# vivek87799/lightweight-human-pose-estimation.pytorch

Hardware: AMD Instinct MI355X
Metric: frames/sec end-to-end (net+grouping) at 368px (higher is better)
Workload: dtype f32; 1 GPU; batch=1 per GPU, 368x656 frames, 1 refinement stage(s), fp32 convs / f32+f64 post, resident normalised NCHW input -> key-points + pose entries on host; 3 frame batch(es) in flight per GPU (3 engine stream(s), each step a complete pass); global_batch=1, parallelism=dp1 (frames sharded, no data-path collective), 3 stream(s) per GPU

## Files before the change

lightweight-human-pose-estimation.pytorch_amd/csrc/net_kernels.hip:

```cpp
#include <cstdio>
#include <cstdlib>

#include <type_traits>
#include "lwp_internal.h"

namespace lwp {

typedef float f32x4 __attribute__((ext_vector_type(4)));
typedef float f32x2 __attribute__((ext_vector_type(2)));
typedef float f32x16 __attribute__((ext_vector_type(16)));

__device__ __forceinline__ float elu_negative(float v) {
    const float p = v * (1.f + v * (0.5f + v * (1.f / 6.f + v * (1.f / 24.f + v * (1.f / 120.f + v * (1.f / 720.f + v * (1.f / 5040.f)))))));
    return v > -0.5f ? p : __expf(v) - 1.0f;
}
__device__ __forceinline__ float apply_act(float v, int act) {
    if (act == ACT_RELU) return fmaxf(v, 0.0f);
    if (act == ACT_ELU) return v > 0.0f ? v : elu_negative(v);
    return v;
}

constexpr int ST_TX = 32;
template <bool BF16, int ST_TY, int PY = 1, int DBG = 0, bool WL = false, bool F16 = false>
__global__ void __launch_bounds__(ST_TY * ST_TX) stem_kernel(StemParams p) {
// ... 1070 lines not shown
                    *(f32x4*)(At + (row0 + i) * ldA + c) = acc;
                }
            } else {
                int xi = xo, yi = yo, im = img;
#pragma unroll
                for (int i = 0; i < PXG; ++i) {
                    const bool ok = m + i < M32;
                    const int yc = yi * p.stride, xc = xi * p.stride;
                    const int base = ((im * p.Hi + yc) * p.Wi + xc) * pix_b + c * 4;
                    f32x4 x[9];
#pragma unroll
                    for (int t = 0; t < 9; ++t) {
                        const int dy = (t / 3 - 1) * p.dil, dx = (t % 3 - 1) * p.dil;
                        const bool in = ok && yc + dy >= 0 && yc + dy < p.Hi && xc + dx >= 0 && xc + dx < p.Wi;
                        x[t] = ldw(in ? (unsigned)(base + dy * row_b + dx * pix_b) : 0x80000000u);
                    }
                    f32x4 acc = bias;
#pragma unroll
                    for (int t = 0; t < 9; ++t) acc += x[t] * wv[t];
                    acc.x = apply_act(acc.x, act_dw); acc.y = apply_act(acc.y, act_dw);
                    acc.z = apply_act(acc.z, act_dw); acc.w = apply_act(acc.w, act_dw);
                    *(f32x4*)(At + (row0 + i) * ldA + c) = acc;
                    if (++xi == Wo) { xi = 0; if (++yi == Ho) { yi = 0; ++im; } }
                }
            }
            m += adv;
            xo += adv_x; yo += adv_y;
            if (xo >= Wo) { xo -= Wo; ++yo; }
            while (yo >= Ho) { yo -= Ho; ++img; }
        }
    }
    __syncthreads();

    f32x4 acc[RT][2];
#pragma unroll
    for (int a = 0; a < RT; ++a) { acc[a][0] = f32x4{0.f, 0.f, 0.f, 0.f}; acc[a][1] = f32x4{0.f, 0.f, 0.f, 0.f}; }
    const float* a_lane = At + r16 * ldA + 4 * q;
    auto one = [&](int step, auto P_) {
        constexpr int P = decltype(P_)::value;
        const int nxt = step + PF - 1 < nsteps ? step + PF - 1 : nsteps - 1;
        if (!(DBG & 2)) load_b(nxt, bw[(P + PF - 1) % PF]);
        __builtin_amdgcn_sched_barrier(0);
        if (DBG & 4) return;
        const f32x4* bcur = bw[P];
#pragma unroll
        for (int u = 0; u < 2; ++u) {
            f32x4 av[RT];
#pragma unroll
            for (int a = 0; a < RT; ++a) av[a] = *(const f32x4*)(a_lane + a * 16 * ldA + step * 32 + 16 * u);
#pragma unroll
            for (int j = 0; j < 4; ++j) {
#pragma unroll
                for (int t = 0; t < 2; ++t) {
                    const int v = u * 8 + j * 2 + t;
                    const float b = bcur[v >> 2][v & 3];
#pragma unroll
                    for (int a = 0; a < RT; ++a) acc[a][t] = __builtin_amdgcn_mfma_f32_16x16x4f32(b, av[a][j], acc[a][t], 0, 0, 0);
                }
            }
        }
    };
    int s0 = 0;
    for (; s0 + PF <= nsteps; s0 += PF) {
        one(s0, std::integral_constant<int, 0>{});
        if (PF > 1) one(s0 + 1, std::integral_constant<int, 1 % PF>{});
        if (PF > 2) one(s0 + 2, std::integral_constant<int, 2 % PF>{});
    }
    if (s0 < nsteps) { one(s0, std::integral_constant<int, 0>{}); ++s0; }
    if (PF > 2 && s0 < nsteps) { one(s0, std::integral_constant<int, 1 % PF>{}); ++s0; }
#pragma unroll
    for (int t = 0; t < 2; ++t) {
        const int n = wave * 32 + t * 16 + 4 * q;
        const f32x4 bias = *(const f32x4*)(p.pw_b + n);
#pragma unroll
        for (int a = 0; a < RT; ++a) {
            const int64_t m = m0 + a * 16 + r16;
            if (m < M) {
                f32x4 v = acc[a][t] + bias;
                v.x = apply_act(v.x, act_pw); v.y = apply_act(v.y, act_pw);
                v.z = apply_act(v.z, act_pw); v.w = apply_act(v.w, act_pw);
                if (p.res) v += *(const f32x4*)(p.res + m * p.res_ld + n);
                *(f32x4*)(p.out + m * p.out_ld + n) = v;
            }
        }
    }
}

template <int BM, int NW, int DBG = 0, int ACT = -1>
static hipError_t launch_dwpw_t(const DwPwParams& p, hipStream_t s) {
    const int64_t M = (int64_t)p.N * p.Ho * p.Wo;
    const size_t lds = (size_t)BM * (p.C + DWPW_F32_APAD) * sizeof(float);
    if ((int64_t)p.N * p.Hi * p.Wi * p.in_ld * 4 >= (1ll << 31)) return hipErrorInvalidValue;
    const int nsplit = (p.cout / 32) / NW;
    static LdsAttrOnce attr;
    if (lds > 48 * 1024) {
        hipError_t e = attr.ensure((const void*)dwpw_kernel<BM, NW, DBG, ACT>, 160 * 1024);
        if (e != hipSuccess) return e;
    }
    hipLaunchKernelGGL((dwpw_kernel<BM, NW, DBG, ACT>), dim3((unsigned)((M + BM - 1) / BM), nsplit), dim3(NW * 64), lds, s, p);
    return hipGetLastError();
}

template <int C>
__global__ void __launch_bounds__(1024) dwpw_pipe_kernel(DwPwParams p, int ntiles) {
    constexpr int BM = 32, NT = 1024, RT = BM / 16, NSTEP = C / 32;
    constexpr int ldA = C + DWPW_F32_APAD;
    constexpr int CG = C / 4;
    constexpr int PAR = NT / CG;
    constexpr int NIT = BM / PAR;
    static_assert(NIT * 4 == NSTEP, "one pixel per four K steps");
    extern __shared__ __attribute__((aligned(16))) float dsm[];
    float* Wd = dsm + 2 * BM * ldA;
    const int tid = threadIdx.x, lane = tid & 63;
    const int wave_u = __builtin_amdgcn_readfirstlane(tid >> 6);
    const int r16 = lane & 15, q = lane >> 4;
    const int M32 = p.N * p.Ho * p.Wo;
    const int G = gridDim.x;
    int bid = blockIdx.x;
    {
        const int qq = G >> 3, rem = G & 7, xcd = bid & 7;
        bid = (xcd < rem ? xcd * (qq + 1) : rem * (qq + 1) + (xcd - rem) * qq) + (bid >> 3);
    }
    for (int i = tid * 4; i < 10 * C; i += NT * 4) *(f32x4*)(Wd + i) = *(const f32x4*)(p.dw_w + i);
    const __amdgpu_buffer_rsrc_t wrsrc = __builtin_amdgcn_make_buffer_rsrc((void*)p.pw_w, 0, 0x7fffffff, 0x00020000);
    const __amdgpu_buffer_rsrc_t irsrc = __builtin_amdgcn_make_buffer_rsrc((void*)p.in, 0, (int)((int64_t)p.N * p.Hi * p.Wi * p.in_ld * 4), 0x00020000);
    const int pix_b = p.in_ld * 4, row_b = p.Wi * pix_b;
    const int c = (tid % CG) * 4, prow = tid / CG;
    constexpr int NU = 16;
    f32x4 bw[2][4];
    auto load_b = [&](int step, f32x4* dst) {
        const unsigned soff = (unsigned)(step * NU + wave_u) * 4096u;
#pragma unroll
        for (int j = 0; j < 4; ++j) dst[j] = __builtin_bit_cast(f32x4, __builtin_amdgcn_raw_buffer_load_b128(wrsrc, lane * 16 + j * 1024, soff, 0));
    };
    f32x4 win[9], pacc;
    auto p_piece = [&](int tl, int it, int j, float* Adst) {
        if (j == 0) {
            const int m = tl * BM + it * PAR + prow;
            const bool ok = m < M32;
            const unsigned q1 = (unsigned)m / (unsigned)p.Wo;
            const int xo = m - (int)q1 * p.Wo;
            const int img = (int)(q1 / (unsigned)p.Ho);
            const int yo = (int)q1 - img * p.Ho;
            const int yc = yo * p.stride, xc = xo * p.stride;
            const int base = ((img * p.Hi + yc) * p.Wi + xc) * pix_b + c * 4;
#pragma unroll
            for (int t = 0; t < 9; ++t) {
                const int dy = (t / 3 - 1) * p.dil, dx = (t % 3 - 1) * p.dil;
                const bool in = ok && yc + dy >= 0 && yc + dy < p.Hi && xc + dx >= 0 && xc + dx < p.Wi;
                win[t] = __builtin_bit_cast(f32x4, __builtin_amdgcn_raw_buffer_load_b128(irsrc, in ? (unsigned)(base + dy * row_b + dx * pix_b) : 0x80000000u, 0, 0));
            }
        } else if (j == 1) {
            pacc = *(const f32x4*)(Wd + 9 * C + c);
#pragma unroll
            for (int t = 0; t < 4; ++t) pacc += win[t] * *(const f32x4*)(Wd + t * C + c);
        } else if (j == 2) {
#pragma unroll
            for (int t = 4; t < 9; ++t) pacc += win[t] * *(const f32x4*)(Wd + t * C + c);
        } else {
            f32x4 v = pacc;
            v.x = fmaxf(v.x, 0.f); v.y = fmaxf(v.y, 0.f); v.z = fmaxf(v.z, 0.f); v.w = fmaxf(v.w, 0.f);
            *(f32x4*)(Adst + (it * PAR + prow) * ldA + c) = v;
        }
    };
    __syncthreads();
    int tile = bid;
    if (tile < ntiles) {
#pragma unroll
        for (int it = 0; it < NIT; ++it)
#pragma unroll
            for (int j = 0; j < 4; ++j) p_piece(tile, it, j, dsm);
    }
    load_b(0, bw[0]);
    __syncthreads();
    int cur = 0;
    for (; tile < ntiles; tile += G) {
        const float* Ac = dsm + cur * BM * ldA;
        float* An = dsm + (cur ^ 1) * BM * ldA;
        const int tnext = tile + G < ntiles ? tile + G : tile;
        f32x4 acc[RT][2];
#pragma unroll
        for (int a = 0; a < RT; ++a) { acc[a][0] = f32x4{0.f, 0.f, 0.f, 0.f}; acc[a][1] = f32x4{0.f, 0.f, 0.f, 0.f}; }
        const float* a_lane = Ac + r16 * ldA + 4 * q;
#pragma unroll
        for (int step = 0; step < NSTEP; ++step) {
            load_b((step + 1) % NSTEP, bw[(step + 1) & 1]);
            __builtin_amdgcn_sched_barrier(0);
            p_piece(tnext, step >> 2, step & 3, An);
            const f32x4* bcur = bw[step & 1];
#pragma unroll
            for (int u = 0; u < 2; ++u) {
                f32x4 av[RT];
#pragma unroll
                for (int a = 0; a < RT; ++a) av[a] = *(const f32x4*)(a_lane + a * 16 * ldA + step * 32 + 16 * u);
#pragma unroll
                for (int j = 0; j < 4; ++j)
#pragma unroll
                    for (int t = 0; t < 2; ++t) {
                        const int v = u * 8 + j * 2 + t;
                        const float b = bcur[v >> 2][v & 3];
#pragma unroll
                        for (int a = 0; a < RT; ++a) acc[a][t] = __builtin_amdgcn_mfma_f32_16x16x4f32(b, av[a][j], acc[a][t], 0, 0, 0);
                    }
            }
        }
        __syncthreads();
        cur ^= 1;
#pragma unroll
        for (int t = 0; t < 2; ++t) {
            const int n = wave_u * 32 + t * 16 + 4 * q;
            const f32x4 bias = *(const f32x4*)(p.pw_b + n);
#pragma unroll
            for (int a = 0; a < RT; ++a) {
                const int m = tile * BM + a * 16 + r16;
                if (m < M32) {
                    f32x4 v = acc[a][t] + bias;
                    v.x = fmaxf(v.x, 0.f); v.y = fmaxf(v.y, 0.f); v.z = fmaxf(v.z, 0.f); v.w = fmaxf(v.w, 0.f);
                    *(f32x4*)(p.out + (int64_t)m * p.out_ld + n) = v;
                }
            }
        }
    }
}

template <int C>
static hipError_t launch_dwpw_pipe_t(const DwPwParams& p, hipStream_t s) {
    const int64_t M = (int64_t)p.N * p.Ho * p.Wo;
    const int ntiles = (int)((M + 31) / 32);
    const size_t lds = (size_t)(2 * 32 * (C + DWPW_F32_APAD) + 10 * C) * sizeof(float);
    static LdsAttrOnce attr;
    hipError_t e = attr.ensure((const void*)dwpw_pipe_kernel<C>, 160 * 1024);
    if (e != hipSuccess) return e;
    int dev = 0, cus = 256;
    if (hipGetDevice(&dev) != hipSuccess || hipDeviceGetAttribute(&cus, hipDeviceAttributeMultiprocessorCount, dev) != hipSuccess || cus <= 0) cus = 256;
    const Tuning& T = p.tune ? *p.tune : default_tuning();
    int grid = cus * (lds <= 80 * 1024 ? 2 : 1);
    if (T.dwpw_pp_grid > 0) grid = T.dwpw_pp_grid;
    if (grid > ntiles) grid = ntiles;
    hipLaunchKernelGGL((dwpw_pipe_kernel<C>), dim3(grid), dim3(1024), lds, s, p, ntiles);
    return hipGetLastError();
}

static hipError_t try_dwpw_pipe(const DwPwParams& p, hipStream_t s, bool* used) {
    *used = false;
    const Tuning& T = p.tune ? *p.tune : default_tuning();
    if (T.dwpw_pipe == 0) return hipSuccess;
    const int64_t M = (int64_t)p.N * p.Ho * p.Wo;
    if (p.cout != 512 || (p.C != 256 && p.C != 512) || p.res || p.act_dw != ACT_RELU || p.act_pw != ACT_RELU) return hipSuccess;
    if ((p.stride != 1 && p.stride != 2) || (p.in_ld & 3) || (p.out_ld & 3) || (((uintptr_t)p.out) & 15) || (((uintptr_t)p.in) & 15)) return hipSuccess;
    if (M >= (1ll << 31) - 64 || (int64_t)p.N * p.Hi * p.Wi * p.in_ld * 4 >= (1ll << 31)) return hipSuccess;
    if (T.dwpw_pipe != 1 && M < 32 * 2048) return hipSuccess;
    if (T.dwpw_pipe != 1 && p.C != 512) return hipSuccess;
    *used = true;
    LWP_VARIANT(p, "dwpw_pipe<%d>", p.C);
    return p.C == 512 ? launch_dwpw_pipe_t<512>(p, s) : launch_dwpw_pipe_t<256>(p, s);
}

bool dwpw_supported(int C, int cout) {
    return C % 32 == 0 && (cout == 64 || cout == 128 || cout == 256 || cout == 512);
}

hipError_t launch_dwpw(const DwPwParams& p_in, hipStream_t s) {
    const DwPwParams& p = p_in;
    {
        bool used = false;
        hipError_t e = try_dwpw_tiled_f32(p, s, &used);
        if (e != hipSuccess || used) return e;
        e = try_dwpw_pipe(p, s, &used);
        if (e != hipSuccess || used) return e;
    }
    const int64_t M = (int64_t)p.N * p.Ho * p.Wo;
    const int nw = p.cout / 32;
    int bm = 16;
    if (M / 32 >= 450) bm = 32;
    if (M / 64 >= 900) bm = 64;
    if (bm == 64 && nw >= 16) bm = 32;
    int nw_wg = nw;
    const Tuning& T = p.tune ? *p.tune : default_tuning();
    if (T.dwpw_bm) bm = T.dwpw_bm;
    if (T.dwpw_nw > 0 && T.dwpw_nw < nw && nw % T.dwpw_nw == 0) nw_wg = T.dwpw_nw;
    if (bm > 64) bm = 64;
    while (bm > 16 && (size_t)bm * (p.C + DWPW_F32_APAD) * sizeof(float) > 150 * 1024) bm >>= 1;
    LWP_VARIANT(p, "dwpw<%d,%d>", bm, nw_wg);
#ifdef LWP_ABLATION
    const int d = T.dwpw_debug;
#define DP_DBG(BM_, NW_, D_) if (bm == BM_ && nw_wg == NW_ && d == D_) return launch_dwpw_t<BM_, NW_, D_>(p, s);
#define DP_DBGS(BM_, NW_) DP_DBG(BM_, NW_, 1) DP_DBG(BM_, NW_, 2) DP_DBG(BM_, NW_, 3) DP_DBG(BM_, NW_, 4) DP_DBG(BM_, NW_, 6) DP_DBG(BM_, NW_, 7) DP_DBG(BM_, NW_, 8)
    DP_DBGS(16, 16) DP_DBGS(16, 8) DP_DBGS(16, 4)
#undef DP_DBGS
#undef DP_DBG
#endif
    const bool relu = p.act_dw == ACT_RELU && p.act_pw == ACT_RELU;
#define DP_CASE(BM_, NW_) if (bm == BM_ && nw_wg == NW_) return relu ? launch_dwpw_t<BM_, NW_, 0, ACT_RELU>(p, s) : launch_dwpw_t<BM_, NW_>(p, s);
    DP_CASE(16, 2) DP_CASE(32, 2) DP_CASE(64, 2)
    DP_CASE(16, 4) DP_CASE(32, 4) DP_CASE(64, 4)
    DP_CASE(16, 8) DP_CASE(32, 8) DP_CASE(64, 8)
    DP_CASE(16, 16) DP_CASE(32, 16) DP_CASE(64, 16)
#undef DP_CASE
    return hipErrorInvalidValue;
}

template <int NW>
__global__ void __launch_bounds__(NW * 64) heads_f32_kernel(HeadsParams p) {
    extern __shared__ __attribute__((aligned(16))) float hsm[];
    const int tid = threadIdx.x, lane = tid & 63;
    const int wave = __builtin_amdgcn_readfirstlane(tid >> 6);
    const int i16 = lane & 15, q = lane >> 4;
    const int M = p.N * p.H * p.W;
    int bid = blockIdx.x;
    {
        const int nwg = gridDim.x, qq = nwg >> 3, rem = nwg & 7, xcd = bid & 7;
        bid = (xcd < rem ? xcd * (qq + 1) : rem * (qq + 1) + (xcd - rem) * qq) + (bid >> 3);
    }
    const int m = bid * 16 + i16;
    const bool mok = m < M;
    const float* in = (const float*)p.in;
    const __amdgpu_buffer_rsrc_t xr = __builtin_amdgcn_make_buffer_rsrc((void*)in, 0, (int)((int64_t)M * p.in_ld * 4), 0x00020000);
    const __amdgpu_buffer_rsrc_t w0r = __builtin_amdgcn_make_buffer_rsrc((void*)p.w0, 0, p.hidden * 128 * 4, 0x00020000);
    const __amdgpu_buffer_rsrc_t w1r = __builtin_amdgcn_make_buffer_rsrc((void*)p.w1, 0, 64 * p.hidden * 4, 0x00020000);
    auto ld = [](const __amdgpu_buffer_rsrc_t& r, unsigned voff, unsigned soff) { return __builtin_bit_cast(f32x4, __builtin_amdgcn_raw_buffer_load_b128(r, voff, soff, 0)); };

    const int ntiles = p.hidden / 16;
    const int my = wave < ntiles ? (ntiles - wave + NW - 1) / NW : 0;
    constexpr int HPF = 3;
    f32x4 w0v[HPF][8], w1v[HPF][4], b0v[HPF];
    const __amdgpu_buffer_rsrc_t b0r = __builtin_amdgcn_make_buffer_rsrc((void*)p.b0, 0, p.hidden * 4, 0x00020000);
    const unsigned w0_lane = (unsigned)(i16 * 128 + 32 * q) * 4u, w1_lane = (unsigned)(i16 * p.hidden + 4 * q) * 4u;
    auto request = [&](int k, f32x4* a, f32x4* b, f32x4* bias) {
        const int ht = wave + (k < my ? k : (my > 0 ? my - 1 : 0)) * NW;
        const int htc = ht < ntiles ? ht : 0;
#pragma unroll
        for (int u = 0; u < 8; ++u) a[u] = ld(w0r, w0_lane + 16u * u, (unsigned)htc * (16u * 128u * 4u));
#pragma unroll
        for (int t = 0; t < 4; ++t) b[t] = ld(w1r, w1_lane + (unsigned)(t * 16 * p.hidden) * 4u, (unsigned)htc * 64u);
        *bias = ld(b0r, 16u * q, (unsigned)htc * 64u);
    };
    request(0, w0v[0], w1v[0], &b0v[0]);
    if (HPF > 2) request(1, w0v[1], w1v[1], &b0v[1]);
    f32x4 xf[8];
#pragma unroll
    for (int u = 0; u < 8; ++u) xf[u] = ld(xr, mok ? (unsigned)((m * p.in_ld + 32 * q + 4 * u) * 4) : 0x80000000u, 0);

    f32x4 acc2[4];
#pragma unroll
    for (int t = 0; t < 4; ++t) acc2[t] = f32x4{0.f, 0.f, 0.f, 0.f};
    const int hsplit = p.out_split > 0 ? p.hidden / 2 : p.hidden;
    const int t_last_lo = p.out_split > 0 ? (p.out_split + 15) / 16 : 4;
    const int t_first_hi = p.out_split > 0 ? p.out_split / 16 : 0;
    auto one = [&](int k, auto P_) {
        constexpr int P = decltype(P_)::value;
        request(k + HPF - 1, w0v[(P + HPF - 1) % HPF], w1v[(P + HPF - 1) % HPF], &b0v[(P + HPF - 1) % HPF]);
        __builtin_amdgcn_sched_barrier(0);
        const f32x4 b0 = b0v[P];
        f32x4 acc1 = {0.f, 0.f, 0.f, 0.f};
#pragma unroll
        for (int u = 0; u < 8; ++u)
#pragma unroll
            for (int c = 0; c < 4; ++c) acc1 = __builtin_amdgcn_mfma_f32_16x16x4f32(w0v[P][u][c], xf[u][c], acc1, 0, 0, 0);
        f32x4 hv;
#pragma unroll
        for (int r = 0; r < 4; ++r) hv[r] = fmaxf(acc1[r] + b0[r], 0.f);
        const int ht = wave + (k < my ? k : 0) * NW;
        const bool first_half = ht * 16 < hsplit;
        const int t_lo = first_half ? 0 : t_first_hi, t_hi = first_half ? t_last_lo : 4;
#pragma unroll
        for (int t = 0; t < 4; ++t) {
            if (t < t_lo || t >= t_hi) continue;
#pragma unroll
            for (int r = 0; r < 4; ++r) acc2[t] = __builtin_amdgcn_mfma_f32_16x16x4f32(w1v[P][t][r], hv[r], acc2[t], 0, 0, 0);
        }
    };
    int k = 0;
    for (; k + HPF <= my; k += HPF) {
        one(k, std::integral_constant<int, 0>{});
        one(k + 1, std::integral_constant<int, 1 % HPF>{});
        if (HPF > 2) one(k + 2, std::integral_constant<int, 2 % HPF>{});
    }
    if (k < my) { one(k, std::integral_constant<int, 0>{}); ++k; }
    if (HPF > 2 && k < my) { one(k, std::integral_constant<int, 1 % HPF>{}); ++k; }

#pragma unroll
    for (int t = 0; t < 4; ++t) *(f32x4*)(hsm + ((wave * 4 + t) * 64 + lane) * 4) = acc2[t];
    __syncthreads();
    if (tid >= 256) return;
    const int t = tid >> 6;
    f32x4 v = *(const f32x4*)(hsm + ((0 * 4 + t) * 64 + lane) * 4);
#pragma unroll
    for (int w = 1; w < NW; ++w) v += *(const f32x4*)(hsm + ((w * 4 + t) * 64 + lane) * 4);
    const int n = 16 * t + 4 * q;
    if (!mok || n >= p.cout) return;
    v += *(const f32x4*)(p.b1 + n);
    float* out = (float*)p.out;
    if (((p.out_ld & 3) == 0) && ((((uintptr_t)out) & 15) == 0) && n + 3 < p.cout) *(f32x4*)(out + (int64_t)m * p.out_ld + n) = v;
    else {
#pragma unroll
        for (int r = 0; r < 4; ++r) if (n + r < p.cout) out[(int64_t)m * p.out_ld + n + r] = v[r];
    }
    if (p.out_nchw || p.out_nchw2) {
        const int HW = p.H * p.W;
        const int img = m / HW, pix = m - img * HW;
        const int c0 = p.out_split > 0 ? p.out_split : p.cout;
#pragma unroll
        for (int r = 0; r < 4; ++r) {
            const int ch = n + r;
            if (ch >= p.cout) continue;
            if (ch < c0) { if (p.out_nchw) p.out_nchw[((int64_t)img * c0 + ch) * HW + pix] = v[r]; }
            else if (p.out_nchw2) p.out_nchw2[((int64_t)img * (p.cout - c0) + (ch - c0)) * HW + pix] = v[r];
        }
    }
}

constexpr int HL_HC = 32, HL_LD0 = 128 + 8, HL_LD1 = HL_HC + 8;
template <int PT>
__global__ void __launch_bounds__(256) heads_f32_lds_kernel(HeadsParams p) {
    extern __shared__ __attribute__((aligned(16))) float hl_sm[];
    float* W0s = hl_sm;
    float* W1s = W0s + 2 * HL_HC * HL_LD0;
    float* B0s = W1s + 2 * 64 * HL_LD1;
    const int tid = threadIdx.x, lane = tid & 63;
    const int wave = __builtin_amdgcn_readfirstlane(tid >> 6);
    const int i16 = lane & 15, q = lane >> 4;
    const int M = p.N * p.H * p.W;
    int bid = blockIdx.x;
    {
        const int nwg = gridDim.x, qq = nwg >> 3, rem = nwg & 7, xcd = bid & 7;
        bid = (xcd < rem ? xcd * (qq + 1) : rem * (qq + 1) + (xcd - rem) * qq) + (bid >> 3);
    }
    int mr[PT];
    bool mok[PT];
#pragma unroll
    for (int i = 0; i < PT; ++i) { mr[i] = bid * (64 * PT) + (wave * PT + i) * 16 + i16; mok[i] = mr[i] < M; }
    const int nch = p.hidden / HL_HC;
    const float* in = (const float*)p.in;
    const __amdgpu_buffer_rsrc_t xr = __builtin_amdgcn_make_buffer_rsrc((void*)in, 0, (int)((int64_t)M * p.in_ld * 4), 0x00020000);
    const __amdgpu_buffer_rsrc_t w0r = __builtin_amdgcn_make_buffer_rsrc((void*)p.w0, 0, p.hidden * 128 * 4, 0x00020000);
    const __amdgpu_buffer_rsrc_t w1r = __builtin_amdgcn_make_buffer_rsrc((void*)p.w1, 0, 64 * p.hidden * 4, 0x00020000);
    auto ld = [](const __amdgpu_buffer_rsrc_t& r, unsigned voff, unsigned soff) { return __builtin_bit_cast(f32x4, __builtin_amdgcn_raw_buffer_load_b128(r, voff, soff, 0)); };
    f32x4 st0[4], st1[2];
    auto request = [&](int c) {
#pragma unroll
        for (int u = 0; u < 4; ++u) {
            const int ch = tid + u * 256, row = ch >> 5, col = (ch & 31) * 4;
            st0[u] = ld(w0r, (unsigned)(row * 128 + col) * 4u, (unsigned)c * (HL_HC * 128 * 4));
        }
#pragma unroll
        for (int u = 0; u < 2; ++u) {
            const int ch = tid + u * 256, row = ch >> 3, col = (ch & 7) * 4;
            st1[u] = ld(w1r, (unsigned)(row * p.hidden + col) * 4u, (unsigned)c * (HL_HC * 4));
        }
    };
    auto land = [&](int buf) {
#pragma unroll
        for (int u = 0; u < 4; ++u) {
            const int ch = tid + u * 256, row = ch >> 5, col = (ch & 31) * 4;
            *(f32x4*)(W0s + (buf * HL_HC + row) * HL_LD0 + col) = st0[u];
        }
#pragma unroll
        for (int u = 0; u < 2; ++u) {
            const int ch = tid + u * 256, row = ch >> 3, col = (ch & 7) * 4;
            *(f32x4*)(W1s + (buf * 64 + row) * HL_LD1 + col) = st1[u];
        }
    };
    request(0);
    f32x4 xf[PT][8];
#pragma unroll
    for (int i = 0; i < PT; ++i)
#pragma unroll
        for (int u = 0; u < 8; ++u) xf[i][u] = ld(xr, mok[i] ? (unsigned)((mr[i] * p.in_ld + 16 * u + 4 * q) * 4) : 0x80000000u, 0);
    for (int i = tid * 4; i < p.hidden; i += 256 * 4) *(f32x4*)(B0s + i) = *(const f32x4*)(p.b0 + i);
    land(0);
    __syncthreads();

    f32x4 acc2[PT][4];
#pragma unroll
    for (int i = 0; i < PT; ++i)
#pragma unroll
        for (int t = 0; t < 4; ++t) acc2[i][t] = f32x4{0.f, 0.f, 0.f, 0.f};
    const int hsplit = p.out_split > 0 ? p.hidden / 2 : p.hidden;
    const int t_last_lo = p.out_split > 0 ? (p.out_split + 15) / 16 : 4;
    const int t_first_hi = p.out_split > 0 ? p.out_split / 16 : 0;
    for (int c = 0; c < nch; ++c) {
        const int buf = c & 1;
        request(c + 1 < nch ? c + 1 : c);
        __builtin_amdgcn_sched_barrier(0);
#pragma unroll
        for (int j = 0; j < HL_HC / 16; ++j) {
            const float* w0 = W0s + (buf * HL_HC + j * 16 + i16) * HL_LD0 + 4 * q;
            f32x4 wv[8];
#pragma unroll
            for (int u = 0; u < 8; ++u) wv[u] = *(const f32x4*)(w0 + 16 * u);
            const f32x4 b0 = *(const f32x4*)(B0s + c * HL_HC + j * 16 + 4 * q);
            const int ht16 = (c * HL_HC + j * 16);
            const bool first_half = ht16 < hsplit;
            const int t_lo = first_half ? 0 : t_first_hi, t_hi = first_half ? t_last_lo : 4;
            f32x4 w1v[4];
#pragma unroll
            for (int t = 0; t < 4; ++t) w1v[t] = *(const f32x4*)(W1s + (buf * 64 + t * 16 + i16) * HL_LD1 + j * 16 + 4 * q);
            __builtin_amdgcn_sched_barrier(0);
            f32x4 acc1[PT];
#pragma unroll
            for (int i = 0; i < PT; ++i) acc1[i] = f32x4{0.f, 0.f, 0.f, 0.f};
#pragma unroll
            for (int u = 0; u < 8; ++u)
#pragma unroll
                for (int cc = 0; cc < 4; ++cc)
#pragma unroll
                    for (int i = 0; i < PT; ++i) acc1[i] = __builtin_amdgcn_mfma_f32_16x16x4f32(wv[u][cc], xf[i][u][cc], acc1[i], 0, 0, 0);
            f32x4 hv[PT];
#pragma unroll
            for (int i = 0; i < PT; ++i)
#pragma unroll
                for (int r = 0; r < 4; ++r) hv[i][r] = fmaxf(acc1[i][r] + b0[r], 0.f);
#pragma unroll
            for (int t = 0; t < 4; ++t) {
                if (t < t_lo || t >= t_hi) continue;
#pragma unroll
                for (int r = 0; r < 4; ++r)
#pragma unroll
                    for (int i = 0; i < PT; ++i) acc2[i][t] = __builtin_amdgcn_mfma_f32_16x16x4f32(w1v[t][r], hv[i][r], acc2[i][t], 0, 0, 0);
            }
        }
        if (c + 1 < nch) land(buf ^ 1);
        __syncthreads();
    }

    float* out = (float*)p.out;
    const int HW = p.H * p.W;
    const int c0 = p.out_split > 0 ? p.out_split : p.cout;
    const bool out_vec = ((p.out_ld & 3) == 0) && ((((uintptr_t)out) & 15) == 0);
#pragma unroll
    for (int i = 0; i < PT; ++i) {
        if (!mok[i]) continue;
        const int m = mr[i];
        const int img = m / HW, pix = m - img * HW;
#pragma unroll
        for (int t = 0; t < 4; ++t) {
            const int n = 16 * t + 4 * q;
            if (n >= p.cout) continue;
            f32x4 v = acc2[i][t];
            v += *(const f32x4*)(p.b1 + n);
            if (out_vec && n + 3 < p.cout) *(f32x4*)(out + (int64_t)m * p.out_ld + n) = v;
            else {
#pragma unroll
                for (int r = 0; r < 4; ++r) if (n + r < p.cout) out[(int64_t)m * p.out_ld + n + r] = v[r];
            }
            if (p.out_nchw || p.out_nchw2) {
#pragma unroll
                for (int r = 0; r < 4; ++r) {
                    const int ch = n + r;
                    if (ch >= p.cout) continue;
                    if (ch < c0) { if (p.out_nchw) p.out_nchw[((int64_t)img * c0 + ch) * HW + pix] = v[r]; }
                    else if (p.out_nchw2) p.out_nchw2[((int64_t)img * (p.cout - c0) + (ch - c0)) * HW + pix] = v[r];
                }
            }
        }
    }
}

bool heads_f32_supported(int cin_pad, int hidden, int cout_pad, int64_t M, const Tuning* tune) {
    const int64_t max_m = (tune && tune->heads_f32_max_m > 0) ? tune->heads_f32_max_m : 4096;
    if (!(cin_pad == 128 && hidden % 16 == 0 && hidden >= 128 && hidden <= 4096 && cout_pad == 64)) return false;
    if (M <= max_m) return true;
    return hidden % HL_HC == 0 && !(tune && tune->heads_f32_lds == 0);
}

hipError_t launch_heads_f32(const HeadsParams& p, hipStream_t s) {
    constexpr int NW = 8;
    const int64_t M = (int64_t)p.N * p.H * p.W;
    if (M * p.in_ld * 4 >= (1ll << 31) || (p.in_ld & 3)) return hipErrorInvalidValue;
    const int64_t max_m = (p.tune && p.tune->heads_f32_max_m > 0) ? p.tune->heads_f32_max_m : 4096;
    if (M > max_m) {
        constexpr int PT = 2;
        if (M >= (1ll << 31) - 64 * PT) return hipErrorInvalidValue;
        const size_t lds2 = (size_t)(2 * HL_HC * HL_LD0 + 2 * 64 * HL_LD1 + p.hidden) * sizeof(float);
        static LdsAttrOnce attr;
        hipError_t e = attr.ensure((const void*)heads_f32_lds_kernel<PT>, 96 * 1024);
        if (e != hipSuccess) return e;
        LWP_VARIANT(p, "heads_f32_lds<%d>", PT);
        hipLaunchKernelGGL(heads_f32_lds_kernel<PT>, dim3((unsigned)((M + 64 * PT - 1) / (64 * PT))), dim3(256), lds2, s, p);
        return hipGetLastError();
    }
    const size_t lds = (size_t)NW * 4 * 64 * 4 * sizeof(float);
    LWP_VARIANT(p, "heads_f32<%d>", NW);
    hipLaunchKernelGGL(heads_f32_kernel<NW>, dim3((unsigned)((M + 15) / 16)), dim3(NW * 64), lds, s, p);
    return hipGetLastError();
}

const Tuning& default_tuning() { static const Tuning t; return t; }
Tuning tuning_from_env() {
    Tuning t;
    auto geti = [](const char* name, int* dst) { const char* e = getenv(name); if (e && e[0]) *dst = atoi(e); };
    auto digit = [](const char* name, int* dst) { const char* e = getenv(name); if (e && e[0]) *dst = e[0] - '0'; };
    geti("LWP_STEM_TY", &t.stem_ty); digit("LWP_STEM_WL", &t.stem_wl); geti("LWP_STEM_DEBUG", &t.stem_debug);
    digit("LWP_DW_TILED", &t.dw_tiled); geti("LWP_DW_CC", &t.dw_cc); geti("LWP_DW_PH", &t.dw_ph);
    digit("LWP_GEMM_WP", &t.gemm_wp);
    if (const char* e = getenv("LWP_GEMM_C3")) t.has_c3 = sscanf(e, "%d,%d,%d", &t.c3[0], &t.c3[1], &t.c3[2]) == 3;
    if (const char* e = getenv("LWP_GEMM_PW")) t.has_pw = sscanf(e, "%d,%d,%d", &t.pw[0], &t.pw[1], &t.pw[2]) == 3;
    geti("LWP_DWPW_BM", &t.dwpw_bm); geti("LWP_DWPW_NW", &t.dwpw_nw); geti("LWP_DWPW_DEBUG", &t.dwpw_debug); geti("LWP_DWPWH_DEBUG", &t.dwpwh_debug);
    digit("LWP_DWPW_PIPE", &t.dwpw_pipe);
    digit("LWP_DWPW_TILED", &t.dwpw_tiled); geti("LWP_DWPW_TILED_WGS", &t.dwpw_tiled_wgs);
    digit("LWP_DWPW_PP", &t.dwpw_pp); geti("LWP_DWPW_PP_GRID", &t.dwpw_pp_grid);
    geti("LWP_HEADS_RM", &t.heads_rm);
    digit("LWP_GEMMH_PERSIST", &t.gemmh_persist); digit("LWP_GEMMH_FOLD", &t.gemmh_fold);
    if (const char* e = getenv("LWP_GEMMH_AR")) {
        if (e[0] == '0' && e[1] == 0) t.gemmh_ar_off = 1;
        else t.has_gemmh_ar = sscanf(e, "%d,%d,%d,%d", &t.gemmh_ar[0], &t.gemmh_ar[1], &t.gemmh_ar[2], &t.gemmh_ar[3]) == 4;
    }
    if (const char* e = getenv("LWP_GEMMH_AR_FORCE")) t.gemmh_ar_force = e[0] == '1';
    geti("LWP_GEMMH_DEBUG", &t.gemmh_debug);
    if (const char* e = getenv("LWP_GEMMH")) t.has_gemmh = sscanf(e, "%d,%d,%d,%d", &t.gemmh[0], &t.gemmh[1], &t.gemmh[2], &t.gemmh[3]) == 4;
    digit("LWP_UPSAMPLE_TILED", &t.upsample_tiled);
    digit("LWP_PEAK_TILE", &t.peak_tile); digit("LWP_PAIR_FORM", &t.pair_form); digit("LWP_POST_NCHW", &t.post_nchw); digit("LWP_HEADS_F32_LDS", &t.heads_f32_lds); digit("LWP_MS_FUSED", &t.ms_fused); digit("LWP_MS_VEC", &t.ms_vec); geti("LWP_MS_TX", &t.ms_tx); digit("LWP_HOST_FETCH_DMA", &t.host_fetch_dma); geti("LWP_DWPW_LDS_PAD", &t.dwpw_lds_pad_kb);
    geti("LWP_HEADS_F32_MAXM", &t.heads_f32_max_m);
    geti("LWP_MAX_FRAMES_PER_PASS", &t.max_frames_per_pass);
    digit("LWP_FUSE_DWPW", &t.fuse_dwpw); digit("LWP_MERGE_HEADS", &t.merge_heads); digit("LWP_FUSE_HEADS", &t.fuse_heads);
    digit("LWP_PRE_BATCH_VEC", &t.pre_batch_vec); digit("LWP_POST_STREAM", &t.post_stream); digit("LWP_POST_GENERIC", &t.post_generic);
    return t;
}

__global__ void __launch_bounds__(256) nchw_from_nhwc_kernel(const float* src, int src_ld, float* dst, int N, int HW, int C) {
    const int64_t total = (int64_t)N * C * HW;
    const int64_t idx = (int64_t)blockIdx.x * blockDim.x + threadIdx.x;
    if (idx >= total) return;
    const int pix = (int)(idx % HW);
    const int64_t t = idx / HW;
    const int c = (int)(t % C);
    const int n = (int)(t / C);
    dst[idx] = src[((int64_t)n * HW + pix) * src_ld + c];
}
hipError_t launch_nchw_from_nhwc(const float* src, int src_ld, float* dst, int N, int HW, int C, hipStream_t s) {
    const int64_t total = (int64_t)N * C * HW;
    hipLaunchKernelGGL(nchw_from_nhwc_kernel, dim3((unsigned)((total + 255) / 256)), dim3(256), 0, s, src, src_ld, dst, N, HW, C);
    return hipGetLastError();
}

}
```

Measured before the change: 2537 frames/s.

## Split heads kernel per output head and process two pixel blocks per workgroup

The small-M fused heads MLP kernel now gives each workgroup 32 pixels (two 16-row blocks) instead of 16, so every weight fragment loaded feeds two MFMA chains. When the output is split into two heads, the grid is doubled and each workgroup handles only its head's hidden tiles and output tiles, so weights are no longer loaded for tiles it skips. The prefetch depth drops from 3 to 2 to make room for the doubled activation and accumulator registers, and the LDS reduction buffer doubles to 64 KB with all 8 waves taking part in the final reduction. The cost is higher register pressure, and in the split case the input rows are read twice, once per head.

Measured after the change: 2569 frames/s, median of 6. 1.01x the previous value.

```diff
diff --git a/lightweight-human-pose-estimation.pytorch_amd/csrc/net_kernels.hip b/lightweight-human-pose-estimation.pytorch_amd/csrc/net_kernels.hip
--- a/lightweight-human-pose-estimation.pytorch_amd/csrc/net_kernels.hip
+++ b/lightweight-human-pose-estimation.pytorch_amd/csrc/net_kernels.hip
@@ -1396,6 +1396,7 @@
 
 template <int NW>
 __global__ void __launch_bounds__(NW * 64) heads_f32_kernel(HeadsParams p) {
+    static_assert(NW == 8, "the reduction maps the 8 waves onto 2 pixel blocks x 4 output tiles");
     extern __shared__ __attribute__((aligned(16))) float hsm[];
     const int tid = threadIdx.x, lane = tid & 63;
     const int wave = __builtin_amdgcn_readfirstlane(tid >> 6);
@@ -1406,89 +1407,105 @@
         const int nwg = gridDim.x, qq = nwg >> 3, rem = nwg & 7, xcd = bid & 7;
         bid = (xcd < rem ? xcd * (qq + 1) : rem * (qq + 1) + (xcd - rem) * qq) + (bid >> 3);
     }
-    const int m = bid * 16 + i16;
-    const bool mok = m < M;
+    const int nheads = p.out_split > 0 ? 2 : 1;
+    const int head = nheads == 2 ? (bid & 1) : 0;
+    const int ptile = nheads == 2 ? (bid >> 1) : bid;
+    int mm[2];
+    bool mok[2];
+#pragma unroll
+    for (int x = 0; x < 2; ++x) { mm[x] = ptile * 32 + x * 16 + i16; mok[x] = mm[x] < M; }
     const float* in = (const float*)p.in;
     const __amdgpu_buffer_rsrc_t xr = __builtin_amdgcn_make_buffer_rsrc((void*)in, 0, (int)((int64_t)M * p.in_ld * 4), 0x00020000);
     const __amdgpu_buffer_rsrc_t w0r = __builtin_amdgcn_make_buffer_rsrc((void*)p.w0, 0, p.hidden * 128 * 4, 0x00020000);
     const __amdgpu_buffer_rsrc_t w1r = __builtin_amdgcn_make_buffer_rsrc((void*)p.w1, 0, 64 * p.hidden * 4, 0x00020000);
     auto ld = [](const __amdgpu_buffer_rsrc_t& r, unsigned voff, unsigned soff) { return __builtin_bit_cast(f32x4, __builtin_amdgcn_raw_buffer_load_b128(r, voff, soff, 0)); };
 
-    const int ntiles = p.hidden / 16;
+    const int ntiles = p.hidden / 16 / nheads;
+    const int ht0 = head * ntiles;
+    const int t_lo = head ? p.out_split / 16 : 0;
+    const int nt = (nheads == 2 && !head ? (p.out_split + 15) / 16 : 4) - t_lo;
+    const int c_lo = head ? p.out_split : 0, c_hi = (nheads == 2 && !head) ? p.out_split : p.cout;
     const int my = wave < ntiles ? (ntiles - wave + NW - 1) / NW : 0;
-    constexpr int HPF = 3;
+    constexpr int HPF = 2;
     f32x4 w0v[HPF][8], w1v[HPF][4], b0v[HPF];
     const __amdgpu_buffer_rsrc_t b0r = __builtin_amdgcn_make_buffer_rsrc((void*)p.b0, 0, p.hidden * 4, 0x00020000);
     const unsigned w0_lane = (unsigned)(i16 * 128 + 32 * q) * 4u, w1_lane = (unsigned)(i16 * p.hidden + 4 * q) * 4u;
     auto request = [&](int k, f32x4* a, f32x4* b, f32x4* bias) {
-        const int ht = wave + (k < my ? k : (my > 0 ? my - 1 : 0)) * NW;
-        const int htc = ht < ntiles ? ht : 0;
+        const int hl = wave + (k < my ? k : (my > 0 ? my - 1 : 0)) * NW;
+        const int htc = ht0 + (hl < ntiles ? hl : 0);
 #pragma unroll
         for (int u = 0; u < 8; ++u) a[u] = ld(w0r, w0_lane + 16u * u, (unsigned)htc * (16u * 128u * 4u));
 #pragma unroll
-        for (int t = 0; t < 4; ++t) b[t] = ld(w1r, w1_lane + (unsigned)(t * 16 * p.hidden) * 4u, (unsigned)htc * 64u);
+        for (int t = 0; t < 4; ++t) {
+            const int to = t_lo + (t < nt ? t : nt - 1);
+            b[t] = ld(w1r, w1_lane, (unsigned)htc * 64u + (unsigned)(to * 16 * p.hidden) * 4u);
+        }
         *bias = ld(b0r, 16u * q, (unsigned)htc * 64u);
     };
     request(0, w0v[0], w1v[0], &b0v[0]);
-    if (HPF > 2) request(1, w0v[1], w1v[1], &b0v[1]);
-    f32x4 xf[8];
-#pragma unroll
-    for (int u = 0; u < 8; ++u) xf[u] = ld(xr, mok ? (unsigned)((m * p.in_ld + 32 * q + 4 * u) * 4) : 0x80000000u, 0);
-
-    f32x4 acc2[4];
-#pragma unroll
-    for (int t = 0; t < 4; ++t) acc2[t] = f32x4{0.f, 0.f, 0.f, 0.f};
-    const int hsplit = p.out_split > 0 ? p.hidden / 2 : p.hidden;
-    const int t_last_lo = p.out_split > 0 ? (p.out_split + 15) / 16 : 4;
-    const int t_first_hi = p.out_split > 0 ? p.out_split / 16 : 0;
+    f32x4 xf[2][8];
+#pragma unroll
+    for (int x = 0; x < 2; ++x)
+#pragma unroll
+        for (int u = 0; u < 8; ++u) xf[x][u] = ld(xr, mok[x] ? (unsigned)((mm[x] * p.in_ld + 32 * q + 4 * u) * 4) : 0x80000000u, 0);
+
+    f32x4 acc2[2][4];
+#pragma unroll
+    for (int x = 0; x < 2; ++x)
+#pragma unroll
+        for (int t = 0; t < 4; ++t) acc2[x][t] = f32x4{0.f, 0.f, 0.f, 0.f};
     auto one = [&](int k, auto P_) {
         constexpr int P = decltype(P_)::value;
         request(k + HPF - 1, w0v[(P + HPF - 1) % HPF], w1v[(P + HPF - 1) % HPF], &b0v[(P + HPF - 1) % HPF]);
         __builtin_amdgcn_sched_barrier(0);
         const f32x4 b0 = b0v[P];
-        f32x4 acc1 = {0.f, 0.f, 0.f, 0.f};
+        f32x4 acc1[2] = {{0.f, 0.f, 0.f, 0.f}, {0.f, 0.f, 0.f, 0.f}};
 #pragma unroll
         for (int u = 0; u < 8; ++u)
 #pragma unroll
-            for (int c = 0; c < 4; ++c) acc1 = __builtin_amdgcn_mfma_f32_16x16x4f32(w0v[P][u][c], xf[u][c], acc1, 0, 0, 0);
-        f32x4 hv;
-#pragma unroll
-        for (int r = 0; r < 4; ++r) hv[r] = fmaxf(acc1[r] + b0[r], 0.f);
-        const int ht = wave + (k < my ? k : 0) * NW;
-        const bool first_half = ht * 16 < hsplit;
-        const int t_lo = first_half ? 0 : t_first_hi, t_hi = first_half ? t_last_lo : 4;
+            for (int c = 0; c < 4; ++c)
+#pragma unroll
+                for (int x = 0; x < 2; ++x) acc1[x] = __builtin_amdgcn_mfma_f32_16x16x4f32(w0v[P][u][c], xf[x][u][c], acc1[x], 0, 0, 0);
+        f32x4 hv[2];
+#pragma unroll
+        for (int x = 0; x < 2; ++x)
+#pragma unroll
+            for (int r = 0; r < 4; ++r) hv[x][r] = fmaxf(acc1[x][r] + b0[r], 0.f);
 #pragma unroll
         for (int t = 0; t < 4; ++t) {
-            if (t < t_lo || t >= t_hi) continue;
-#pragma unroll
-            for (int r = 0; r < 4; ++r) acc2[t] = __builtin_amdgcn_mfma_f32_16x16x4f32(w1v[P][t][r], hv[r], acc2[t], 0, 0, 0);
+            if (t >= nt) continue;
+#pragma unroll
+            for (int r = 0; r < 4; ++r)
+#pragma unroll
+                for (int x = 0; x < 2; ++x) acc2[x][t] = __builtin_amdgcn_mfma_f32_16x16x4f32(w1v[P][t][r], hv[x][r], acc2[x][t], 0, 0, 0);
         }
     };
     int k = 0;
     for (; k + HPF <= my; k += HPF) {
         one(k, std::integral_constant<int, 0>{});
-        one(k + 1, std::integral_constant<int, 1 % HPF>{});
-        if (HPF > 2) one(k + 2, std::integral_constant<int, 2 % HPF>{});
-    }
-    if (k < my) { one(k, std::integral_constant<int, 0>{}); ++k; }
-    if (HPF > 2 && k < my) { one(k, std::integral_constant<int, 1 % HPF>{}); ++k; }
-
-#pragma unroll
-    for (int t = 0; t < 4; ++t) *(f32x4*)(hsm + ((wave * 4 + t) * 64 + lane) * 4) = acc2[t];
+        one(k + 1, std::integral_constant<int, 1>{});
+    }
+    if (k < my) one(k, std::integral_constant<int, 0>{});
+
+#pragma unroll
+    for (int x = 0; x < 2; ++x)
+#pragma unroll
+        for (int t = 0; t < 4; ++t) *(f32x4*)(hsm + (((wave * 2 + x) * 4 + t) * 64 + lane) * 4) = acc2[x][t];
     __syncthreads();
-    if (tid >= 256) return;
-    const int t = tid >> 6;
-    f32x4 v = *(const f32x4*)(hsm + ((0 * 4 + t) * 64 + lane) * 4);
-#pragma unroll
-    for (int w = 1; w < NW; ++w) v += *(const f32x4*)(hsm + ((w * 4 + t) * 64 + lane) * 4);
-    const int n = 16 * t + 4 * q;
-    if (!mok || n >= p.cout) return;
+    const int x = wave >> 2, t = wave & 3;
+    if (t >= nt) return;
+    f32x4 v = *(const f32x4*)(hsm + (((0 * 2 + x) * 4 + t) * 64 + lane) * 4);
+#pragma unroll
+    for (int w = 1; w < NW; ++w) v += *(const f32x4*)(hsm + (((w * 2 + x) * 4 + t) * 64 + lane) * 4);
+    const int n = 16 * (t_lo + t) + 4 * q;
+    const int m = x ? mm[1] : mm[0];
+    if (!(x ? mok[1] : mok[0]) || n >= c_hi || n + 3 < c_lo) return;
     v += *(const f32x4*)(p.b1 + n);
     float* out = (float*)p.out;
-    if (((p.out_ld & 3) == 0) && ((((uintptr_t)out) & 15) == 0) && n + 3 < p.cout) *(f32x4*)(out + (int64_t)m * p.out_ld + n) = v;
+    if (((p.out_ld & 3) == 0) && ((((uintptr_t)out) & 15) == 0) && n >= c_lo && n + 3 < c_hi) *(f32x4*)(out + (int64_t)m * p.out_ld + n) = v;
     else {
 #pragma unroll
-        for (int r = 0; r < 4; ++r) if (n + r < p.cout) out[(int64_t)m * p.out_ld + n + r] = v[r];
+        for (int r = 0; r < 4; ++r) if (n + r >= c_lo && n + r < c_hi) out[(int64_t)m * p.out_ld + n + r] = v[r];
     }
     if (p.out_nchw || p.out_nchw2) {
         const int HW = p.H * p.W;
@@ -1497,7 +1514,7 @@
 #pragma unroll
         for (int r = 0; r < 4; ++r) {
             const int ch = n + r;
-            if (ch >= p.cout) continue;
+            if (ch < c_lo || ch >= c_hi) continue;
             if (ch < c0) { if (p.out_nchw) p.out_nchw[((int64_t)img * c0 + ch) * HW + pix] = v[r]; }
             else if (p.out_nchw2) p.out_nchw2[((int64_t)img * (p.cout - c0) + (ch - c0)) * HW + pix] = v[r];
         }
@@ -1674,9 +1691,14 @@
         hipLaunchKernelGGL(heads_f32_lds_kernel<PT>, dim3((unsigned)((M + 64 * PT - 1) / (64 * PT))), dim3(256), lds2, s, p);
         return hipGetLastError();
     }
-    const size_t lds = (size_t)NW * 4 * 64 * 4 * sizeof(float);
+    const size_t lds = (size_t)NW * 2 * 4 * 64 * 4 * sizeof(float);
+    const unsigned nheads = p.out_split > 0 ? 2u : 1u;
+    if (p.out_split < 0 || p.out_split >= p.cout || (nheads == 2 && p.hidden % 32)) return hipErrorInvalidValue;
+    static LdsAttrOnce attr8;
+    hipError_t e = attr8.ensure((const void*)heads_f32_kernel<NW>, 64 * 1024);
+    if (e != hipSuccess) return e;
     LWP_VARIANT(p, "heads_f32<%d>", NW);
-    hipLaunchKernelGGL(heads_f32_kernel<NW>, dim3((unsigned)((M + 15) / 16)), dim3(NW * 64), lds, s, p);
+    hipLaunchKernelGGL(heads_f32_kernel<NW>, dim3((unsigned)((M + 31) / 32) * nheads), dim3(NW * 64), lds, s, p);
     return hipGetLastError();
 }
 
```
